# loganmcbroom/Flan

Measured on AMD Instinct MI355X. Metric: PV analysis+resynthesis frames/sec (2048-win, hop 512, 48 kHz) at 1/2/4/8 GPU, higher is better.
Workload: dtype f32; 1 GPU; 8 ch x 60 s x 48 kHz uniform noise per GPU, convert_to_PV(2048,512,dft 2048) -> convert_to_audio round trip; channels_per_gpu=8, parallelism=channel-shard x1

## Files before the change

flan_amd/__init__.py:

```python
import ctypes as C
import os

import numpy as np

_HERE = os.path.dirname(os.path.abspath(__file__))
LIB_PATH = os.environ.get("FLAN_AMD_LIB") or os.path.join(_HERE, "libflanhip.so")

OK, ERR_INVALID_ARG, ERR_UNSUPPORTED, ERR_HIP, ERR_CANCELLED, ERR_NO_DEVICE = 0, -1, -2, -3, -4, -5


class FlanHipError(RuntimeError):
    def __init__(self, code, message):
        super().__init__("flanhip error %d: %s" % (code, message))
        self.code = code


if not os.path.exists(LIB_PATH):
    raise ImportError("flan_amd/libflanhip.so is missing: build it with `python flan_amd/build.py` "
                      "(hipcc --offload-arch=gfx950); there is no fallback path")

lib = C.CDLL(LIB_PATH)

_f32p = np.ctypeslib.ndpointer(np.float32, flags="C_CONTIGUOUS")
_vp, _i64, _i32, _f32 = C.c_void_p, C.c_int64, C.c_int, C.c_float
# ... 14 lines not shown
    "flanhip_touch_pages": (C.c_int, [_vp, C.c_size_t]),
    "flanhip_host_workers": (C.c_int, []),
    "flanhip_parallel_for": (C.c_int, [C.c_int, _vp, _vp]),
    "flanhip_stream_create": (C.c_int, [C.POINTER(_vp)]),
    "flanhip_stream_destroy": (C.c_int, [_vp]),
    "flanhip_host_malloc": (C.c_int, [C.POINTER(_vp), C.c_size_t]),
    "flanhip_host_free": (C.c_int, [_vp]),
    "flanhip_memcpy_h2d": (C.c_int, [_vp, _vp, C.c_size_t, _vp]),
    "flanhip_memcpy_d2h": (C.c_int, [_vp, _vp, C.c_size_t, _vp]),
    "flanhip_memset": (C.c_int, [_vp, _i32, C.c_size_t, _vp]),
    "flanhip_stream_synchronize": (C.c_int, [_vp]),
    "flanhip_wait_cancellable": (C.c_int, [_vp, _vp]),
    "flanhip_wait_cancellable_fn": (C.c_int, [_vp, _vp, _vp]),
    "flanhip_analyze": (C.c_int, [_vp, _i64, _i64, _f32, _i32, _i32, _i32, _vp, C.POINTER(_i64), _vp]),
    "flanhip_analyze_dev": (C.c_int, [_vp, _i64, _i64, _f32, _i32, _i32, _i32, _vp, _vp]),
    "flanhip_synthesize": (C.c_int, [_vp, _i64, _i64, _i32, _f32, _f32, _i32, _vp, C.POINTER(_i32), _vp]),
    "flanhip_synthesize_workspace_bytes": (C.c_size_t, [_i64, _i64, _i32, _f32, _f32, _i32]),
    "flanhip_synthesize_dev": (C.c_int, [_vp, _i64, _i64, _i32, _f32, _f32, _i32, _vp, _vp, _vp, _vp]),
    "flanhip_analyze_dev_fused": (C.c_int, [_vp, _i64, _i64, _f32, _i32, _i32, _i32, _vp, _vp, _vp]),
    "flanhip_synthesize_dev_fused": (C.c_int, [_vp, _i64, _i64, _i32, _f32, _f32, _i32, _vp, _vp, _vp, _vp]),
    "flanhip_synthesize_dev_stages": (C.c_int, [_vp, _i64, _i64, _i32, _f32, _f32, _i32, _vp, _vp, _vp, _i32, _i32, _vp]),
    "flanhip_debug_option": (None, [_i32, _i32]),
    "flanhip_debug_kernel_scratch_bytes": (_i32, [_i32]),
    "flanhip_modify_time": (C.c_int, [_vp, _i64, _i64, _i32, _f32, _i32, _vp, _i64, _vp, _vp]),
    "flanhip_modify_time_dev": (C.c_int, [_vp, _i64, _i64, _i32, _f32, _i32, _vp, _i64, _vp, _vp]),
    "flanhip_modify_time_dev_fused": (C.c_int, [_vp, _i64, _i64, _i32, _f32, _f32, _vp, _i64, _vp, _i32, _vp, _vp]),
    "flanhip_synthesize_dev_fused_checked": (C.c_int, [_vp, _i64, _i64, _i32, _f32, _f32, _i32, _vp, _vp, _vp, _vp]),
    "flanhip_stretch_map_dev": (C.c_int, [_vp, _i64, _i32, _f32, _i32, _vp, _vp]),
    "flanhip_stretch_map_const_dev": (C.c_int, [_f32, _vp, _i64, _i32, _f32, _i32, _vp, _vp]),
    "flanhip_fill_dev": (C.c_int, [_vp, _i64, _f32, _vp]),
    "flanhip_modify_frequency": (C.c_int, [_vp, _i64, _i64, _i32, _f32, _vp, _vp, _vp, _vp]),
    "flanhip_modify_frequency_dev": (C.c_int, [_vp, _i64, _i64, _i32, _f32, _vp, _vp, _vp, _vp]),
    "flanhip_modify_time_interp_dev": (C.c_int, [_vp, _i64, _i64, _i32, _f32, _i32, _vp, _i64, _i32, _vp, _vp]),
    "flanhip_modify_time_interp_dev_fused": (C.c_int, [_vp, _i64, _i64, _i32, _f32, _f32, _vp, _i64, _i32, _vp, _i32, _vp, _vp]),
    "flanhip_modify_frequency_interp_dev": (C.c_int, [_vp, _i64, _i64, _i32, _f32, _vp, _vp, _i32, _vp, _vp]),
    "flanhip_repitch_interp_dev": (C.c_int, [_vp, _i64, _i64, _i32, _f32, _vp, _i32, _vp, _vp]),
    "flanhip_repitch_map_dev": (C.c_int, [_vp, _i64, _i64, _i32, _f32, _vp, _vp, _vp]),
    "flanhip_repitch_dev": (C.c_int, [_vp, _i64, _i64, _i32, _f32, _vp, _vp, _vp]),
    "flanhip_shape_affine": (C.c_int, [_vp, _i64, _i64, _i32, _f32, _f32, _f32, _f32, _f32, _i32, _vp, _vp]),
    "flanhip_shape_affine_dev": (C.c_int, [_vp, _i64, _i64, _i32, _f32, _f32, _f32, _f32, _f32, _i32, _vp, _vp]),
    "flanhip_shape_table_dev": (C.c_int, [_vp, _vp, _i64, _i64, _i32, _f32, _i32, _vp, _vp]),
    "flanhip_replace_amplitudes_dev": (C.c_int, [_vp, _i64, _i64, _i32, _vp, _i64, _i64, _i32, _vp, _f32, _vp, _vp]),
    "flanhip_subtract_amplitudes_dev": (C.c_int, [_vp, _i64, _i64, _i32, _vp, _i64, _i64, _i32, _vp, _f32, _vp, _vp]),
    "flanhip_resonate_out_frames": (_i64, [_i64, _f32, _f32, _i32]),
    "flanhip_resonate_dev": (C.c_int, [_vp, _i64, _i64, _i32, _f32, _i32, _i64, _vp, _f32, _vp, _vp]),
    "flanhip_n_loudest_partials_dev": (C.c_int, [_vp, _i64, _i64, _i32, _vp, C.c_int32, _i32, _vp, _vp]),
# ... 441 lines not shown


def analyze_dev(d_audio, ch, n, sample_rate, window, hop, dft, d_out, stream=None):
    check(lib.flanhip_analyze_dev(_dp(d_audio), ch, n, sample_rate, window, hop, dft, _dp(d_out), _vp(stream or 0)))


def analyze_dev_fused(d_audio, ch, n, sample_rate, window, hop, dft, d_out, d_ws, stream=None):
    check(lib.flanhip_analyze_dev_fused(_dp(d_audio), ch, n, sample_rate, window, hop, dft, _dp(d_out), _dp(d_ws), _vp(stream or 0)))


def synthesize_dev_fused(d_pv, ch, F, bins, sample_rate, analysis_rate, window, d_out, d_ws, d_nan=None, stream=None):
    check(lib.flanhip_synthesize_dev_fused(_dp(d_pv), ch, F, bins, sample_rate, analysis_rate, window, _dp(d_out), _dp(d_ws),
                                           _dp(d_nan), _vp(stream or 0)))


def synthesize_dev_stages(d_pv, ch, F, bins, sample_rate, analysis_rate, window, d_out, d_ws, d_nan, presummed, stages, stream=None):
    check(lib.flanhip_synthesize_dev_stages(_dp(d_pv), ch, F, bins, sample_rate, analysis_rate, window, _dp(d_out), _dp(d_ws),
                                            _dp(d_nan), presummed, stages, _vp(stream or 0)))


DEBUG_CHAIN_LEN, DEBUG_TARGET_CHAINS, DEBUG_FORCE_GENERIC, DEBUG_NO_FAST_DIV = 0, 1, 2, 3
DEBUG_ANA_VARIANT, DEBUG_SYN_VARIANT, DEBUG_ANA4096_OLD, DEBUG_SYN4096_OLD, DEBUG_RESAMPLE_DIRECT, DEBUG_FORCE_DIRECT, DEBUG_INLINE_FIXUP, DEBUG_WIDE_OFFSETS = 4, 5, 6, 7, 8, 9, 10, 11
_DEBUG_NAMES = {"chain_len": 0, "target_chains": 1, "force_generic": 2, "no_fast_div": 3, "ana_variant": 4, "syn_variant": 5,
                "ana4096_old": 6, "syn4096_old": 7, "resample_direct": 8, "force_direct": 9, "inline_fixup": 10, "wide_offsets": 11, "no_sub": 12}


class debug_options:

    def __init__(self, **kw):
        self.kw = {_DEBUG_NAMES[k]: int(v) for k, v in kw.items()}

    def __enter__(self):
        for k, v in self.kw.items():
            lib.flanhip_debug_option(k, v)
        return self

    def __exit__(self, *exc):
        for k in self.kw:
            lib.flanhip_debug_option(k, 0)
        return False


def synthesize_workspace_bytes(ch, F, bins, sample_rate, analysis_rate, window):
    return int(lib.flanhip_synthesize_workspace_bytes(ch, F, bins, sample_rate, analysis_rate, window))


def synthesize_dev(d_pv, ch, F, bins, sample_rate, analysis_rate, window, d_out, d_ws, d_nan=None, stream=None):
# ... 101 lines not shown
```

flan_amd/csrc/conversions.hip:

```cpp
#include "flanhip_internal.h"
#include <atomic>
#include <memory>
#include "pv_kernels.h"
#include "pv_kernels_fast.h"
#include <type_traits>
#include "pv_kernels_v2.h"
#include "pv_kernels_v3.h"
#include "pv_kernels_eo.h"
#include "pv_kernels_any.h"
#include "pv_kernels_mr.h"
#include "pv_kernels_bs.h"
#include "pv_kernels_big.h"
#include "team_launch.h"
#include "sub_launch.h"
#include <algorithm>
#include <cstdlib>

namespace flanhip {


static constexpr size_t kMaxLds = 160 * 1024;

static constexpr int kMaxAnyDft = 1 << 20;
static bool fft_size( int dft ) { return is_pow2( dft ) && dft >= 32 && dft <= 8192; }
// ... 404 lines not shown
			case 256:  return wbig ? run_synth_eo_team<4, 1, true>( p, tb, s ) : run_synth_eo_team<4, 1>( p, tb, s );
			case 512:  return wbig ? run_synth_eo_team<4, 2, true>( p, tb, s ) : run_synth_eo_team<4, 2>( p, tb, s );
			case 1024: return wbig ? run_synth_eo_team<4, 4, true>( p, tb, s ) : run_synth_eo_team<4, 4>( p, tb, s );
			}
		return FLANHIP_ERR_UNSUPPORTED;
		}
	}

static bool synth_fast_ok( int dft, int W, int hop ) { return synth_fast_kind( dft, W, hop ) != 0; }

static int self_carry_group( int dft, int W, int hop, int chains_per_channel )
	{
	if( sub_shape( dft, W, hop ) ) return chains_per_channel < 128 ? 0 : sub_group_size( dft );
	const int kind = synth_fast_kind( dft, W, hop );
	int g = 0;
	if( kind == 2 ) g = dft == 4096 ? ( debug_options().ana11_old ? 0 : 4 ) : group_size_of( dft );
	else if( kind != 1 ) return 0;
	else if( dft == 2048 || v3_size( dft ) ) g = group_size_of( dft );
	else if( dft == 4096 && !debug_options().ana11_old ) g = 4;
	if( chains_per_channel < 128 ) g = 0;
	return g;
	}

static int launch_analyze_body( const float * d_audio, int64_t ch, int64_t n, float sr, int W, int hop, int dft, flanhip_MF * d_out, void * d_fused_ws, hipStream_t s, bool * left_group_sums, int * epoch );

int launch_analyze( const float * d_audio, int64_t ch, int64_t n, float sr, int W, int hop, int dft, flanhip_MF * d_out, void * d_fused_ws, hipStream_t s )
	{
	bool left_group_sums = false;
	int epoch = 0;
	if( d_fused_ws ) note_workspace_producer( d_fused_ws, 0 );
	const int rc = launch_analyze_body( d_audio, ch, n, sr, W, hop, dft, d_out, d_fused_ws, s, &left_group_sums, &epoch );
	if( !rc && d_fused_ws && left_group_sums ) note_workspace_producer( d_fused_ws, 1, epoch );
	return rc;
	}

static int launch_analyze_body( const float * d_audio, int64_t ch, int64_t n, float sr, int W, int hop, int dft, flanhip_MF * d_out, void * d_fused_ws, hipStream_t s, bool * left_group_sums, int * epoch )
	{
	FLANHIP_REQUIRE( d_audio && d_out, FLANHIP_ERR_INVALID_ARG, "null buffer" );
	FLANHIP_REQUIRE( ch > 0 && n >= 0 && W >= 2 && hop >= 1 && sr > 0.0f, FLANHIP_ERR_INVALID_ARG, "bad sizes" );
	FLANHIP_REQUIRE( W <= dft, FLANHIP_ERR_INVALID_ARG, "window_size larger than dft_size" );
	FLANHIP_REQUIRE( dft_size_ok( dft ), FLANHIP_ERR_UNSUPPORTED, "dft_size must be even, at least 4 and at most 2^20" );
	if( int rc = require_device() ) return rc;
	const bool team = team_shape( dft, W, hop ) && n >= 2 && n < ( int64_t( 1 ) << 31 ) - 65536;
	const bool sub = sub_shape( dft, W, hop ) && n >= 2 && n < ( int64_t( 1 ) << 31 ) - 8192;
	MrPlan mr_plan{};
	const bool mr = !team && mr_size( dft, W, &mr_plan );
	BsPlan bs_plan{};
	const bool bs = !team && !mr && bs_size( dft, W, &bs_plan );
	BigPlan big_plan{};
	const bool big = !team && !mr && !bs && big_size( dft, W, &big_plan );
	const bool any = !team && !fft_size( dft ) && !mr && !bs && !big;
	std::shared_ptr<const PlanRef> plan_ref;
	if( int rc = get_plan( W, dft, &plan_ref ) ) return rc;
	const Plan * plan = &plan_ref->plan;

	AnalyzeParams p{};
	p.audio = d_audio; p.out = reinterpret_cast<MF*>( d_out );
	p.window = plan->d_window; p.tw = plan->d_tw; p.tw2 = plan->d_tw2; p.dump = plan->d_dump;
	p.n = n; p.F = n / hop + 1;
	p.num_channels = int( ch ); p.window_size = W; p.hop = hop;
	const bool fast = ( dft == 2048 || ( dft == 4096 && !debug_options().ana11_old ) || v3_size( dft ) ) && n >= 2 && n < ( int64_t( 1 ) << 31 ) - 8192 && hop <= 65536 && !force_generic();
	int target_chains = team ? team_target_chains( dft ) : sub ? sub_target_chains( dft ) : any ? any_target_chains( dft / 2 + 1 ) : mr ? mr_target_chains( dft, W ) : bs ? bs_target_chains( dft, W ) : big ? big_target_chains() : fast ? fast_target_chains( dft, false ) : generic_target_chains( dft );
	const int block_group = team ? team_group_size( dft ) : sub ? sub_group_size( dft ) : fast ? group_size_of( dft ) : 1;
	p.L = choose_chain_length( ch, p.F, any ? 7 : 1, target_chains, block_group );
	p.chains_per_channel = int( ( p.F + p.L - 1 ) / p.L );
	p.sample_rate = sr;
	p.analysis_rate = sr / hop;
	DivPlan dp;
	if( int rc = get_div_plan( p.analysis_rate, &dp ) ) return rc;
	p.ar_div = DivC{ dp.c, dp.rc, dp.exact };
	p.sums = nullptr; p.nan_out = nullptr; p.nan_epoch = 0;
	p.cancel = thread_cancel_word( s );
	bool kernel_sums = !any && !big && ( !mr || mr_pingpong( mr_plan.C ) ) && ( !bs || bs_pingpong( bs_plan.M ) );
	SynthLayout fused_lay{};
	if( d_fused_ws )
		{
		SynthLayout & lay = fused_lay;
		if( int rc = synth_layout( ch, p.F, dft / 2 + 1, sr, p.analysis_rate, W, &lay ) ) return rc;
		p.nan_epoch = next_epoch();
		*epoch = p.nan_epoch;
		if( kernel_sums && lay.L >= p.L + 8 && int64_t( p.chains_per_channel ) * ch <= target_chains ) kernel_sums = false;
		if( kernel_sums )
			{
			p.L = lay.L;
			p.chains_per_channel = lay.chains_per_channel;
			p.sums = reinterpret_cast<double*>( d_fused_ws );
			p.nan_out = reinterpret_cast<int*>( reinterpret_cast<char*>( d_fused_ws ) + lay.carry_bytes + lay.head_bytes );
			}
		const bool groups_too = ( fast || sub ) && kernel_sums && self_carry_group( dft, W, hop, lay.chains_per_channel ) != 0;
		p.group_sums = groups_too ? reinterpret_cast<double*>( reinterpret_cast<char*>( d_fused_ws ) + lay.group_offset ) : nullptr;
		p.groups_per_channel = lay.groups_per_channel;
		*left_group_sums = groups_too;
		}
	auto prepass_on_behalf = [&]() -> int
		{
		if( !d_fused_ws || kernel_sums ) return FLANHIP_OK;
		SynthParams q{};
		q.pv = reinterpret_cast<const MF*>( d_out );
		q.carry = reinterpret_cast<double*>( d_fused_ws );
		q.F = p.F; q.num_channels = int( ch ); q.num_bins = dft / 2 + 1;
		q.L = fused_lay.L; q.chains_per_channel = fused_lay.chains_per_channel;
		q.analysis_rate = p.analysis_rate; q.ar_div = p.ar_div;
		q.nan_words = reinterpret_cast<int*>( reinterpret_cast<char*>( d_fused_ws ) + fused_lay.carry_bytes + fused_lay.head_bytes );
		q.nan_epoch = p.nan_epoch;
		const int64_t chains = int64_t( q.chains_per_channel ) * ch;
		hipLaunchKernelGGL( k_phase_sums2, dim3( (unsigned) chains, (unsigned) ( ( q.num_bins + 255 ) / 256 ) ), dim3( 256 ), 0, s, q );
		FLANHIP_CHECK( hipGetLastError() );
		return FLANHIP_OK;
		};

	if( team ) { if( int rc = run_analyze_team( p, *plan, dft, s ) ) return rc; return prepass_on_behalf(); }
	if( sub ) { if( int rc = run_analyze_sub( p, dft, s ) ) return rc; return prepass_on_behalf(); }
	if( any )
		{
		std::shared_ptr<const UnitRef> unit_ref;
// ... 97 lines not shown
	FLANHIP_REQUIRE( dft_size_ok( o->dft ), FLANHIP_ERR_UNSUPPORTED, "dft size must be even, at least 4 and at most 2^20" );
	FLANHIP_REQUIRE( int64_t( o->dft ) * W < ( int64_t( 1 ) << 31 ), FLANHIP_ERR_UNSUPPORTED, "dft_size * window_size overflows the int product of AudioPV.cpp:99" );
	const bool team = team_shape( o->dft, W, o->hop );
	const bool sub = sub_shape( o->dft, W, o->hop );
	const bool mr = !team && mr_size( o->dft, W );
	const bool bs = !team && !mr && bs_size( o->dft, W );
	BigPlan big_plan{};
	o->big = !team && !mr && !bs && big_size( o->dft, W, &big_plan );
	o->any = !team && !fft_size( o->dft ) && !mr && !bs && !o->big;
	o->head_len = o->any ? 0 : std::max( W - o->hop, 0 );
	const int overlap = ( W + o->hop - 1 ) / o->hop;
	const int kind = ( o->any || o->big || sub ) ? 0 : synth_fast_kind( o->dft, W, o->hop );
	const int slots = team ? team_target_chains( o->dft ) : sub ? sub_target_chains( o->dft ) : o->any ? any_target_chains( bins ) : mr ? mr_target_chains( o->dft, W ) : bs ? bs_target_chains( o->dft, W ) : o->big ? big_target_chains() : kind == 0 ? generic_target_chains( o->dft ) : fast_target_chains( o->dft, true );
	const int block_group = team ? team_group_size( o->dft ) : sub ? sub_group_size( o->dft ) : kind != 0 ? group_size_of( o->dft ) : 1;
	o->L = choose_chain_length( ch, F, o->any ? 1 : std::max( overlap - 1, 1 ), slots, block_group );
	o->chains_per_channel = int( ( F + o->L - 1 ) / o->L );
	const int64_t chains = int64_t( o->chains_per_channel ) * ch;
	o->carry_bytes = ( size_t( chains ) * bins * sizeof( double ) + 255 ) & ~size_t( 255 );
	o->head_bytes = ( size_t( chains ) * o->head_len * sizeof( float ) + 255 ) & ~size_t( 255 );
	const int gsize = o->any ? 8 : sub ? sub_group_size( o->dft ) : group_size_of( o->dft );
	o->groups_per_channel = ( o->chains_per_channel + gsize - 1 ) / gsize;
	o->group_offset = o->carry_bytes + o->head_bytes + 1024;
	o->group_bytes = ( size_t( ch ) * o->groups_per_channel * bins * sizeof( double ) + 255 ) & ~size_t( 255 );
	o->total_bytes = o->group_offset + 2 * o->group_bytes;
	o->fix_offset = o->tail_offset = 0;
	if( ( team || ( !o->any && !mr && ( o->dft == 2048 || v3_size( o->dft ) || o->dft == 4096 ) && kind == 1 ) ) && o->head_len > 0 )
		{
		o->fix_offset = o->total_bytes;
		o->tail_offset = o->fix_offset + ( ( size_t( chains ) * 8 * sizeof( int ) + 255 ) & ~size_t( 255 ) );
		o->total_bytes = o->tail_offset + o->head_bytes;
		}
	o->any_spec_offset = o->any_frames_offset = 0;
	if( o->any )
		{
		o->any_spec_offset = o->total_bytes;
		o->any_frames_offset = o->any_spec_offset + ( ( size_t( ch ) * size_t( F ) * size_t( bins ) * sizeof( cf ) + 255 ) & ~size_t( 255 ) );
		o->total_bytes = o->any_frames_offset + ( ( size_t( ch ) * size_t( F ) * size_t( W ) * sizeof( float ) + 255 ) & ~size_t( 255 ) );
		}
	o->bsg_offset = 0;
	if( BsPlan bp{}; bs && bs_size( o->dft, W, &bp ) && bp.glob )
		{
		o->bsg_offset = o->total_bytes;
		o->total_bytes += bsg_block_bytes( bp.C, bp.M, W ) * size_t( chains );
		}
	o->mr_ring_offset = 0;
	if( MrPlan mp{}; mr && mr_size( o->dft, W, &mp ) && mp.ring_ws )
		{
// ... 55 lines not shown
	p.window_scale = 2.67f / ( lay.dft * W / lay.hop );
	DivPlan dp;
	if( int rc = get_div_plan( ar, &dp ) ) return rc;
	p.ar_div = DivC{ dp.c, dp.rc, dp.exact };
	p.dump = reinterpret_cast<float*>( reinterpret_cast<char*>( d_ws ) + lay.carry_bytes + lay.head_bytes + 512 );
	p.nan_in = ( presummed == 1 || presummed == 2 ) ? reinterpret_cast<const int*>( reinterpret_cast<char*>( d_ws ) + lay.carry_bytes + lay.head_bytes ) : nullptr;
	p.skip_words = presummed == 2 ? p.nan_in : nullptr;
	p.carry_in = d_carry_in; p.total_out = d_total_out; p.total_only = prepass_only ? 1 : 0;
	p.cancel = thread_cancel_word( s );
	const int fix_hook = debug_options().inline_fixup;
	const bool self_fix = lay.fix_offset != 0 && !prepass_only && ( stage_mask & 0xF ) == 0xF && fix_hook != 2
		&& ( fix_hook == 1 || lay.L >= ( lay.head_len + lay.hop - 1 ) / lay.hop + 3 );
	if( self_fix )
		{
		p.fix_state = reinterpret_cast<int*>( reinterpret_cast<char*>( d_ws ) + lay.fix_offset );
		p.tail = reinterpret_cast<float*>( reinterpret_cast<char*>( d_ws ) + lay.tail_offset );
		p.fix_tag = int( ( unsigned( next_epoch() ) & 0x1FFFFFFFu ) << 2 );
		}

	const int64_t chains = int64_t( p.chains_per_channel ) * ch;
	FLANHIP_REQUIRE( chains < ( int64_t( 1 ) << 31 ), FLANHIP_ERR_UNSUPPORTED, "too many chains for one launch" );
	const int stages = prepass_only ? 3 : ( stage_mask & 0xF );
	int noted_epoch = 0;
	const bool self_carry = presummed == 1 && !prepass_only && !d_carry_in && !d_total_out && debug_options().syn_variant != 2
		&& self_carry_group( lay.dft, W, lay.hop, lay.chains_per_channel ) != 0 && workspace_producer( d_ws, &noted_epoch ) == 1;
	if( self_carry )
		{
		p.expect_epoch = noted_epoch;
		p.group_sums = reinterpret_cast<const double*>( reinterpret_cast<char*>( d_ws ) + lay.group_offset );
		p.groups_per_channel = lay.groups_per_channel;
		const bool scan_groups = p.groups_per_channel > 40;
		p.group_carry = scan_groups ? reinterpret_cast<double*>( reinterpret_cast<char*>( d_ws ) + lay.group_offset + lay.group_bytes ) : nullptr;
		if( scan_groups && ( stages & 2 ) )
			{
			if( p.groups_per_channel <= 512 ) hipLaunchKernelGGL( ( k_phase_scan2<16, true> ), dim3( (unsigned) ( ( bins + 31 ) / 32 ), (unsigned) ch ), dim3( 512 ), 0, s, p );
			else hipLaunchKernelGGL( ( k_phase_scan2<32, true> ), dim3( (unsigned) ( ( bins + 15 ) / 16 ), (unsigned) ch ), dim3( 512 ), 0, s, p );
			FLANHIP_CHECK( hipGetLastError() );
			}
		}
	const int gsize = self_carry_group( lay.dft, W, lay.hop, lay.chains_per_channel );
	const bool group_kernel = !self_carry && gsize != 0 && stages == 0xF && !prepass_only && !d_carry_in && !d_total_out && debug_options().syn_variant != 2 && presummed != 3;
	const bool sums_in_group_kernel = group_kernel && presummed != 1;
	if( ( stages & 1 ) && presummed != 1 && presummed != 3 && !sums_in_group_kernel )
		{
		hipLaunchKernelGGL( k_phase_sums2, dim3( (unsigned) chains, (unsigned) ( ( bins + 255 ) / 256 ) ), dim3( 256 ), 0, s, p );
		FLANHIP_CHECK( hipGetLastError() );
		}
	if( group_kernel )
		{
		double * gs = reinterpret_cast<double*>( reinterpret_cast<char*>( d_ws ) + lay.group_offset );
		p.groups_per_channel = lay.groups_per_channel;
		const dim3 grid( (unsigned) ( ( bins + 255 ) / 256 ), (unsigned) lay.groups_per_channel, (unsigned) ch );
		FLANHIP_REQUIRE( lay.groups_per_channel <= 65535 && ch <= 65535, FLANHIP_ERR_UNSUPPORTED, "too many groups / channels for one launch" );
		if( sums_in_group_kernel ) { if( gsize == 32 ) hipLaunchKernelGGL( k_sums_and_groups<32>, grid, dim3( 256 ), 0, s, p, gs ); else if( gsize == 16 ) hipLaunchKernelGGL( k_sums_and_groups<16>, grid, dim3( 256 ), 0, s, p, gs ); else if( gsize == 8 ) hipLaunchKernelGGL( k_sums_and_groups<8>, grid, dim3( 256 ), 0, s, p, gs ); else hipLaunchKernelGGL( k_sums_and_groups<4>, grid, dim3( 256 ), 0, s, p, gs ); }
		else if( gsize == 32 ) hipLaunchKernelGGL( k_group_sums<32>, grid, dim3( 256 ), 0, s, p, gs ); else if( gsize == 16 ) hipLaunchKernelGGL( k_group_sums<16>, grid, dim3( 256 ), 0, s, p, gs ); else if( gsize == 8 ) hipLaunchKernelGGL( k_group_sums<8>, grid, dim3( 256 ), 0, s, p, gs ); else hipLaunchKernelGGL( k_group_sums<4>, grid, dim3( 256 ), 0, s, p, gs );
// ... 222 lines not shown
	{
	FLANHIP_REQUIRE( presummed >= 0 && presummed <= 2, FLANHIP_ERR_INVALID_ARG, "presummed: 0, 1 or 2" );
	return launch_synthesize( d_pv, ch, F, bins, sr, ar, W, d_out, d_ws, d_nan, presummed, (hipStream_t) stream, nullptr, nullptr, false, stages );
	}

void flanhip_debug_option( int which, int value )
	{
	DebugOptions & o = debug_options();
	switch( which )
		{
		case FLANHIP_DEBUG_CHAIN_LEN:       o.chain_len = value; break;
		case FLANHIP_DEBUG_TARGET_CHAINS:   o.target_chains = value; break;
		case FLANHIP_DEBUG_FORCE_GENERIC:   o.force_generic = value; break;
		case FLANHIP_DEBUG_NO_FAST_DIV:     o.no_fast_div = value; break;
		case FLANHIP_DEBUG_ANA_VARIANT:     o.ana_variant = value; break;
		case FLANHIP_DEBUG_SYN_VARIANT:     o.syn_variant = value; break;
		case FLANHIP_DEBUG_ANA4096_OLD:     o.ana11_old = value; break;
		case FLANHIP_DEBUG_SYN4096_OLD:     o.syn11_old = value; break;
		case FLANHIP_DEBUG_RESAMPLE_DIRECT: o.resample_direct = value; break;
		case FLANHIP_DEBUG_FORCE_DIRECT:    o.force_direct = value; break;
		case FLANHIP_DEBUG_INLINE_FIXUP:    o.inline_fixup = value; break;
		case FLANHIP_DEBUG_WIDE_OFFSETS:    o.wide_offsets = value; break;
		case FLANHIP_DEBUG_NO_SUB:          o.no_sub = value; break;
		default: break;
		}
	}
#ifdef FLANHIP_STAMPS
int flanhip_debug_read_stamps( unsigned long long * out16 )
	{
	FLANHIP_CHECK( hipDeviceSynchronize() );
	FLANHIP_CHECK( hipMemcpyFromSymbol( out16, HIP_SYMBOL( g_stamp_acc ), 16 * sizeof( unsigned long long ) ) );
	unsigned long long zero[16] = { 0 };
	FLANHIP_CHECK( hipMemcpyToSymbol( HIP_SYMBOL( g_stamp_acc ), zero, sizeof( zero ) ) );
	return FLANHIP_OK;
	}
int flanhip_debug_read_spans( unsigned long long * out8192 )
	{
	FLANHIP_CHECK( hipDeviceSynchronize() );
	FLANHIP_CHECK( hipMemcpyFromSymbol( out8192, HIP_SYMBOL( g_stamp_span ), 8192 * sizeof( unsigned long long ) ) );
	return FLANHIP_OK;
	}
#endif

size_t flanhip_synthesize_workspace_bytes( int64_t ch, int64_t F, int bins, float sr, float ar, int W )
	{
	SynthLayout lay;
	if( synth_layout( ch, F, bins, sr, ar, W, &lay ) ) return 0;
	size_t bytes = lay.total_bytes;
// ... 50 lines not shown
```

flan_amd/csrc/flanhip_internal.h:

```cpp
#pragma once
#include <hip/hip_runtime.h>
#include <cstdarg>
#include <cstdint>
#include <cstdio>
#include <cmath>
#include <map>
#include <memory>
#include <mutex>
#include <tuple>
#include <vector>

#include "flanhip.h"
#include "cf_type.h"

namespace flanhip {

void set_error( const char * fmt, ... );

#define FLANHIP_CHECK( expr )                                                                         \
	do { hipError_t e_ = ( expr );                                                                    \
		if( e_ != hipSuccess ) {                                                                      \
			::flanhip::set_error( "%s failed: %s (%s:%d)", #expr, hipGetErrorString( e_ ), __FILE__, __LINE__ ); \
			return FLANHIP_ERR_HIP; } } while( 0 )

// ... 25 lines not shown
inline int team_radix( int dft_size ) { return dft_size == 8192 ? 4 : dft_size == 16384 ? 8 : 0; }
struct TeamTableLayout { int tw1, tw3, twj, tws, two, total; };
inline TeamTableLayout team_table_layout( int R ) { TeamTableLayout l; l.tw1 = 0; l.tw3 = 240; l.twj = 1008; l.tws = l.twj + ( R - 1 ) * 512; l.two = l.tws + ( R / 2 ) * 512; l.total = l.two + 2 * R; return l; }
struct PlanRef { Plan plan; PlanRef() = default; PlanRef( const PlanRef & ) = delete; PlanRef & operator=( const PlanRef & ) = delete; ~PlanRef(); };
int get_plan( int window_size, int dft_size, std::shared_ptr<const PlanRef> * out );

struct DivPlan { float c, rc; int exact; };
int get_div_plan( float c, DivPlan * out );

int choose_chain_length( int64_t num_channels, int64_t num_frames, int min_len, int target_chains, int group = 1 );
struct DebugOptions
	{
	int chain_len = 0;
	int target_chains = 0;
	int force_generic = 0;
	int no_fast_div = 0;
	int ana_variant = 0, syn_variant = 0;
	int ana11_old = 0, syn11_old = 0;
	int resample_direct = 0;
	int wide_offsets = 0;
	int inline_fixup = 0;
	int no_sub = 0;
	int force_direct = 0;
	};
DebugOptions & debug_options();
bool force_generic();
int cu_count();

int launch_analyze( const float * d_audio, int64_t ch, int64_t n, float sr, int W, int hop, int dft, flanhip_MF * d_out, void * d_fused_ws, hipStream_t s );
int launch_synthesize( const flanhip_MF * d_pv, int64_t ch, int64_t F, int bins, float sr, float ar, int W, float * d_out,
	void * d_ws, int * d_nan, int presummed, hipStream_t s, const double * d_carry_in = nullptr, double * d_total_out = nullptr,
	bool prepass_only = false, int stage_mask = 0xF );

int next_epoch();

struct SynthLayout { int hop, dft, L, chains_per_channel, head_len, groups_per_channel; size_t carry_bytes, head_bytes, group_offset, group_bytes, total_bytes;
	size_t flags_offset;
	size_t fix_offset, tail_offset;
	bool any; size_t any_spec_offset, any_frames_offset;
	size_t mr_ring_offset;
	size_t bsg_offset;
	bool big; size_t big_out_offset, big_head_offset, big_ring_offset; };
void note_workspace_producer( const void * d_ws, int kind, int epoch = 0 );
int workspace_producer( const void * d_ws, int * epoch = nullptr );
int synth_layout( int64_t ch, int64_t F, int bins, float sr, float ar, int W, SynthLayout * out );

bool valid_interp( int kind );
float interp_eval_host( int kind, float x );
int processors_set_interp_lut( int slot, const float * d_table );
int processors_ext_set_interp_lut( int slot, const float * d_table );
int processors_arrange_set_interp_lut( int slot, const float * d_table );

}
```

flan_amd/csrc/pv_kernels.h:

```cpp
#pragma once
#include <hip/hip_runtime.h>
#include <stdint.h>
#include "fft_device.h"
#include "pv_math.h"

namespace flanhip {

struct MF { float m, f; };


struct AnalyzeParams
	{
	const float * audio;
	MF * out;
	const float * window;
	const cf * tw;
	const cf * tw2;
	int64_t n;
	int64_t F;
	int num_channels;
	int window_size;
	int hop;
	int L;
	int chains_per_channel;
	float sample_rate;
	float analysis_rate;
	DivC ar_div;
	double * sums;
	int * nan_out;
	int nan_epoch;
	double * group_sums;
	int groups_per_channel;
	const int * cancel;
	float * dump;
	};

__device__ __forceinline__ int cancel_peek( const int * word )
	{
	return word ? __hip_atomic_load( word, __ATOMIC_RELAXED, __HIP_MEMORY_SCOPE_SYSTEM ) : 0;
	}
__device__ __forceinline__ bool cancel_seen( int peeked ) { return __builtin_amdgcn_readfirstlane( peeked ) != 0; }

__device__ __forceinline__ MF phase_vocode_bin( float re, float im, float & prev_phase, float bin_frequency, float expected_phase_diff,
	float analysis_rate, bool use_wrapping )
	{
	const float phase = atan2_fast( im, re );
	const float phase_diff = phase - prev_phase;
	prev_phase = phase;
	const float delta_phase = phase_diff - expected_phase_diff;
	const float wrapped = use_wrapping ? delta_phase - FLANHIP_PI2_F * round_half_away( div_pi2( delta_phase ) ) : delta_phase;
	const float delta_frequency = div_pi2( wrapped * analysis_rate );
	MF r;
	r.m = magnitude_scaled( re, im );
	r.f = bin_frequency + delta_frequency;
	return r;
	}

// ... 440 lines not shown
```

flan_amd/csrc/pv_kernels_v2.h:

```cpp
#pragma once
#include "pv_kernels_fast.h"

namespace flanhip {

struct V2Lds
	{
	static constexpr int C = 1024;
	static constexpr int TW1 = 0;
	static constexpr int TW3 = TW1 + 240;
	static constexpr int W2H = TW3 + 768;
	static constexpr int WIN = W2H + 512;
	static constexpr int KC = WIN + 1024;
	static constexpr int BUF = KC + 1024;
	static constexpr int BUF_LEN = C + C / 16 + 1;
	static constexpr size_t bytes( int waves ) { return size_t( BUF + waves * BUF_LEN ) * 8; }
	};


#ifdef FLANHIP_STAMPS
__device__ unsigned long long g_stamp_acc[16];
__device__ unsigned long long g_stamp_span[2 * 4096];
struct Stamps
	{
	unsigned long long last, acc[12], t_begin, r_begin;
// ... 46 lines not shown
			const unsigned w = blockIdx.x * ( blockDim.x >> 6 ) + ( threadIdx.x >> 6 );
			if( w < 4096 ) { g_stamp_span[2 * w] = r_begin; g_stamp_span[2 * w + 1] = r_end; }
			}
		}
#endif
	};
#else
struct Stamps
	{
	__device__ __forceinline__ void init() {}
	__device__ __forceinline__ void operator()( int ) const {}
	__device__ __forceinline__ void flush( int ) {}
	};
#endif


#ifndef FLANHIP_PUBLISH_DRAIN
#define FLANHIP_PUBLISH_DRAIN 1
#endif
__device__ __forceinline__ void publish_drain()
	{
	if constexpr( FLANHIP_PUBLISH_DRAIN != 0 ) asm volatile( "s_waitcnt vmcnt(0)" ::: "memory" );
	else asm volatile( "" ::: "memory" );
	}

template<int WAVES, bool SUMS, int NV, int ABL = 0>
__global__ __launch_bounds__( 64 * WAVES ) void k_analyze_v2( AnalyzeParams p, FastTables tb )
	{
	using L = V2Lds;
	constexpr int C = 1024, E = 16, H = 8, NT = 64 * WAVES;
	constexpr int NP = NV / 2;
	static_assert( NV == 2 || NV == 4 || NV == 8 || NV == 16, "1, 2, 4 or 8 pairs at a time" );
	typedef float VB __attribute__(( ext_vector_type( NV ) ));
	extern __shared__ __attribute__((aligned(16))) unsigned char smem[];
	cf * s = reinterpret_cast<cf*>( smem );
	const int tid = threadIdx.x, lane = tid & 63, wave = tid >> 6;
	const int W = p.window_size, hop = p.hop;
	const int cancel_word = cancel_peek( p.cancel );

	for( int i = tid; i < 240; i += NT ) s[L::TW1 + i] = tb.tw1[i];
	for( int i = tid; i < 768; i += NT ) s[L::TW3 + i] = tb.tw3[i];
	for( int i = tid; i < 512; i += NT ) { const cf w = tb.w2[i]; s[L::W2H + i] = mk( 0.5f * w.x, 0.5f * w.y ); }
		{
		float * win = reinterpret_cast<float*>( s + L::WIN );
		for( int i = tid; i < 2 * C; i += NT ) win[i] = ( i < W ) ? p.window[i] : 0.0f;
		v4f_t * kc = reinterpret_cast<v4f_t*>( s + L::KC );
// ... 310 lines not shown
				}
			const double vx = fold( sumx );
			if( lane == 0 ) { dst[C / 2] = vx; stage[C / 2] = vx; }
			}
		const bool any_bad = __any( bad );
		if( p.nan_out && lane == 0 && active )
			{
			if( chain == 0 ) { p.nan_out[2] = p.nan_epoch; p.nan_out[4] = p.nan_epoch; }
			if( any_bad ) p.nan_out[0] = p.nan_epoch;
			}
		if( p.group_sums )
			{
			__syncthreads();
			const int live = min( WAVES, p.chains_per_channel - group * WAVES );
			double * gdst = p.group_sums + ( int64_t( channel ) * groups + group ) * ( C + 1 );
			for( int bin = tid; bin <= C; bin += NT )
				{
				double run = 0.0;
				for( int w = 0; w < live; ++w )
					{
					const double v = run + reinterpret_cast<const double*>( s + L::BUF + w * L::BUF_LEN )[bin];
					run = ( __builtin_fabs( v ) < FLANHIP_FOLD_FAST_LIMIT ) ? fold_phase_fast( v ) : fold_phase_any( v );
					}
				gdst[bin] = run;
				}
			}
		}
	}

__device__ __forceinline__ void st_agent( cf * p, cf v )
	{
	unsigned long long bits; __builtin_memcpy( &bits, &v, 8 );
	__hip_atomic_store( reinterpret_cast<unsigned long long*>( p ), bits, __ATOMIC_RELAXED, __HIP_MEMORY_SCOPE_AGENT );
	}
__device__ __forceinline__ cf ld_agent( const cf * p )
	{
	const unsigned long long bits = __hip_atomic_load( reinterpret_cast<const unsigned long long*>( p ), __ATOMIC_RELAXED, __HIP_MEMORY_SCOPE_AGENT );
	cf v; __builtin_memcpy( &v, &bits, 8 );
	return v;
	}

struct V2LdsSyn
	{
	static constexpr int C = 1024;
	static constexpr int TW1 = 0;
	static constexpr int TW3 = TW1 + 240;
	static constexpr int W2S = TW3 + 768;
// ... 464 lines not shown
```

include/flanhip.h:

```cpp
#ifndef FLANHIP_H
#define FLANHIP_H

#include <stddef.h>
#include <stdint.h>

#ifdef __cplusplus
extern "C" {
#endif

#define FLANHIP_OK                 0
#define FLANHIP_ERR_INVALID_ARG   -1
#define FLANHIP_ERR_UNSUPPORTED   -2
#define FLANHIP_ERR_HIP           -3
#define FLANHIP_ERR_CANCELLED     -4
#define FLANHIP_ERR_NO_DEVICE     -5

typedef struct flanhip_MF { float m; float f; } flanhip_MF;

int          flanhip_version(void);
const char * flanhip_last_error(void);
int          flanhip_device_count(void);
int          flanhip_set_device(int device);
int          flanhip_get_device(int * device);

// ... 42 lines not shown
                                 float sample_rate, float analysis_rate, int window_size,
                                 float * d_out, void * d_workspace, int * d_nan_flag, void * stream);
int flanhip_synthesize_dev_fused_checked(const flanhip_MF * d_pv, int64_t num_channels, int64_t num_pv_frames, int num_bins,
                                         float sample_rate, float analysis_rate, int window_size,
                                         float * d_out, void * d_workspace, int * d_nan_flag, void * stream);

int flanhip_synthesize_dev_stages(const flanhip_MF * d_pv, int64_t num_channels, int64_t num_pv_frames, int num_bins,
                                  float sample_rate, float analysis_rate, int window_size,
                                  float * d_out, void * d_workspace, int * d_nan_flag, int presummed, int stages, void * stream);

#define FLANHIP_DEBUG_CHAIN_LEN       0
#define FLANHIP_DEBUG_TARGET_CHAINS   1
#define FLANHIP_DEBUG_FORCE_GENERIC   2
#define FLANHIP_DEBUG_NO_FAST_DIV     3
#define FLANHIP_DEBUG_ANA_VARIANT     4
#define FLANHIP_DEBUG_SYN_VARIANT     5
#define FLANHIP_DEBUG_ANA4096_OLD     6
#define FLANHIP_DEBUG_SYN4096_OLD     7
#define FLANHIP_DEBUG_RESAMPLE_DIRECT 8
#define FLANHIP_DEBUG_FORCE_DIRECT    9
#define FLANHIP_DEBUG_INLINE_FIXUP   10
#define FLANHIP_DEBUG_WIDE_OFFSETS   11
#define FLANHIP_DEBUG_NO_SUB         12
void flanhip_debug_option(int which, int value);
int flanhip_debug_kernel_scratch_bytes(int which);

int flanhip_modify_time(const flanhip_MF * pv, int64_t num_channels, int64_t num_pv_frames, int num_bins,
                        float sample_rate, int hop, const float * mod_seconds,
                        int64_t out_frames, flanhip_MF * out, volatile int * cancel);
int flanhip_modify_time_dev(const flanhip_MF * d_pv, int64_t num_channels, int64_t num_pv_frames, int num_bins,
                            float sample_rate, int hop, const float * d_mod_seconds,
                            int64_t out_frames, flanhip_MF * d_out, void * stream);
int flanhip_modify_time_dev_fused(const flanhip_MF * d_pv, int64_t num_channels, int64_t num_pv_frames, int num_bins,
                                  float sample_rate, float analysis_rate, const float * d_mod, int64_t out_frames,
                                  flanhip_MF * d_out, int window_size, void * d_workspace, void * stream);
int flanhip_stretch_map_dev(float * d_factor, int64_t num_pv_frames, int num_bins, float sample_rate, int hop,
                            float * d_max, void * stream);
int flanhip_stretch_map_const_dev(float factor, float * d_map, int64_t num_pv_frames, int num_bins, float sample_rate, int hop,
                                  float * d_max, void * stream);
int flanhip_fill_dev(float * d_grid, int64_t count, float value, void * stream);

int flanhip_modify_frequency(const flanhip_MF * pv, int64_t num_channels, int64_t num_pv_frames, int num_bins,
                             float sample_rate, const float * mod_hz, const float * in_modified,
                             flanhip_MF * out, volatile int * cancel);
int flanhip_modify_frequency_dev(const flanhip_MF * d_pv, int64_t num_channels, int64_t num_pv_frames, int num_bins,
                                 float sample_rate, const float * d_mod_hz, const float * d_in_modified,
                                 flanhip_MF * d_out, void * stream);
// ... 152 lines not shown
```

Measured before the change: 168.9 million frames/s.

## Compute group phase carries in last analysis block via per-channel ticket

For dft 2048 fast path, the analysis kernel now publishes group phase sums with agent-scope stores, and a per-channel atomic ticket (epoch-tagged) picks the last-finishing block. That block scans the group sums into the carry buffer, so synthesis can skip its separate phase-scan kernel when the producer marks the workspace as carrying group carries. This trades an extra kernel launch and pass for a serial tail scan by one block per channel plus atomics and drains in analysis.

New measurement: 151.5 million frames/s. -10.3%, worse.

```diff
diff --git a/flan_amd/__init__.py b/flan_amd/__init__.py
--- a/flan_amd/__init__.py
+++ b/flan_amd/__init__.py
@@ -60,6 +60,7 @@
     "flanhip_synthesize_dev_stages": (C.c_int, [_vp, _i64, _i64, _i32, _f32, _f32, _i32, _vp, _vp, _vp, _i32, _i32, _vp]),
     "flanhip_debug_option": (None, [_i32, _i32]),
     "flanhip_debug_kernel_scratch_bytes": (_i32, [_i32]),
+    "flanhip_debug_group_layout": (C.c_int, [_i64, _i64, _i32, _f32, _f32, _i32, C.POINTER(_i64)]),
     "flanhip_modify_time": (C.c_int, [_vp, _i64, _i64, _i32, _f32, _i32, _vp, _i64, _vp, _vp]),
     "flanhip_modify_time_dev": (C.c_int, [_vp, _i64, _i64, _i32, _f32, _i32, _vp, _i64, _vp, _vp]),
     "flanhip_modify_time_dev_fused": (C.c_int, [_vp, _i64, _i64, _i32, _f32, _f32, _vp, _i64, _vp, _i32, _vp, _vp]),
@@ -547,7 +548,7 @@
 DEBUG_CHAIN_LEN, DEBUG_TARGET_CHAINS, DEBUG_FORCE_GENERIC, DEBUG_NO_FAST_DIV = 0, 1, 2, 3
 DEBUG_ANA_VARIANT, DEBUG_SYN_VARIANT, DEBUG_ANA4096_OLD, DEBUG_SYN4096_OLD, DEBUG_RESAMPLE_DIRECT, DEBUG_FORCE_DIRECT, DEBUG_INLINE_FIXUP, DEBUG_WIDE_OFFSETS = 4, 5, 6, 7, 8, 9, 10, 11
 _DEBUG_NAMES = {"chain_len": 0, "target_chains": 1, "force_generic": 2, "no_fast_div": 3, "ana_variant": 4, "syn_variant": 5,
-                "ana4096_old": 6, "syn4096_old": 7, "resample_direct": 8, "force_direct": 9, "inline_fixup": 10, "wide_offsets": 11, "no_sub": 12}
+                "ana4096_old": 6, "syn4096_old": 7, "resample_direct": 8, "force_direct": 9, "inline_fixup": 10, "wide_offsets": 11, "no_sub": 12, "group_carry": 13}
 
 
 class debug_options:
diff --git a/flan_amd/csrc/conversions.hip b/flan_amd/csrc/conversions.hip
--- a/flan_amd/csrc/conversions.hip
+++ b/flan_amd/csrc/conversions.hip
@@ -450,19 +450,19 @@
 	return g;
 	}
 
-static int launch_analyze_body( const float * d_audio, int64_t ch, int64_t n, float sr, int W, int hop, int dft, flanhip_MF * d_out, void * d_fused_ws, hipStream_t s, bool * left_group_sums, int * epoch );
+static int launch_analyze_body( const float * d_audio, int64_t ch, int64_t n, float sr, int W, int hop, int dft, flanhip_MF * d_out, void * d_fused_ws, hipStream_t s, int * left_group_sums, int * epoch );
 
 int launch_analyze( const float * d_audio, int64_t ch, int64_t n, float sr, int W, int hop, int dft, flanhip_MF * d_out, void * d_fused_ws, hipStream_t s )
 	{
-	bool left_group_sums = false;
+	int left_group_sums = 0;
 	int epoch = 0;
 	if( d_fused_ws ) note_workspace_producer( d_fused_ws, 0 );
 	const int rc = launch_analyze_body( d_audio, ch, n, sr, W, hop, dft, d_out, d_fused_ws, s, &left_group_sums, &epoch );
-	if( !rc && d_fused_ws && left_group_sums ) note_workspace_producer( d_fused_ws, 1, epoch );
+	if( !rc && d_fused_ws && left_group_sums ) note_workspace_producer( d_fused_ws, left_group_sums, epoch );
 	return rc;
 	}
 
-static int launch_analyze_body( const float * d_audio, int64_t ch, int64_t n, float sr, int W, int hop, int dft, flanhip_MF * d_out, void * d_fused_ws, hipStream_t s, bool * left_group_sums, int * epoch )
+static int launch_analyze_body( const float * d_audio, int64_t ch, int64_t n, float sr, int W, int hop, int dft, flanhip_MF * d_out, void * d_fused_ws, hipStream_t s, int * left_group_sums, int * epoch )
 	{
 	FLANHIP_REQUIRE( d_audio && d_out, FLANHIP_ERR_INVALID_ARG, "null buffer" );
 	FLANHIP_REQUIRE( ch > 0 && n >= 0 && W >= 2 && hop >= 1 && sr > 0.0f, FLANHIP_ERR_INVALID_ARG, "bad sizes" );
@@ -497,7 +497,7 @@
 	DivPlan dp;
 	if( int rc = get_div_plan( p.analysis_rate, &dp ) ) return rc;
 	p.ar_div = DivC{ dp.c, dp.rc, dp.exact };
-	p.sums = nullptr; p.nan_out = nullptr; p.nan_epoch = 0;
+	p.sums = nullptr; p.nan_out = nullptr; p.nan_epoch = 0; p.group_carry = nullptr; p.group_ticket = nullptr;
 	p.cancel = thread_cancel_word( s );
 	bool kernel_sums = !any && !big && ( !mr || mr_pingpong( mr_plan.C ) ) && ( !bs || bs_pingpong( bs_plan.M ) );
 	SynthLayout fused_lay{};
@@ -518,7 +518,10 @@
 		const bool groups_too = ( fast || sub ) && kernel_sums && self_carry_group( dft, W, hop, lay.chains_per_channel ) != 0;
 		p.group_sums = groups_too ? reinterpret_cast<double*>( reinterpret_cast<char*>( d_fused_ws ) + lay.group_offset ) : nullptr;
 		p.groups_per_channel = lay.groups_per_channel;
-		*left_group_sums = groups_too;
+		const bool carries_too = groups_too && fast && dft == 2048 && debug_options().group_carry == 0;
+		p.group_carry = carries_too ? reinterpret_cast<double*>( reinterpret_cast<char*>( d_fused_ws ) + lay.group_offset + lay.group_bytes ) : nullptr;
+		p.group_ticket = carries_too ? reinterpret_cast<unsigned long long*>( reinterpret_cast<char*>( d_fused_ws ) + lay.ticket_offset ) : nullptr;
+		*left_group_sums = groups_too ? ( carries_too ? 2 : 1 ) : 0;
 		}
 	auto prepass_on_behalf = [&]() -> int
 		{
@@ -662,7 +665,8 @@
 	o->groups_per_channel = ( o->chains_per_channel + gsize - 1 ) / gsize;
 	o->group_offset = o->carry_bytes + o->head_bytes + 1024;
 	o->group_bytes = ( size_t( ch ) * o->groups_per_channel * bins * sizeof( double ) + 255 ) & ~size_t( 255 );
-	o->total_bytes = o->group_offset + 2 * o->group_bytes;
+	o->ticket_offset = o->group_offset + 2 * o->group_bytes;
+	o->total_bytes = o->ticket_offset + ( ( size_t( ch ) * sizeof( unsigned long long ) + 255 ) & ~size_t( 255 ) );
 	o->fix_offset = o->tail_offset = 0;
 	if( ( team || ( !o->any && !mr && ( o->dft == 2048 || v3_size( o->dft ) || o->dft == 4096 ) && kind == 1 ) ) && o->head_len > 0 )
 		{
@@ -764,15 +768,18 @@
 	FLANHIP_REQUIRE( chains < ( int64_t( 1 ) << 31 ), FLANHIP_ERR_UNSUPPORTED, "too many chains for one launch" );
 	const int stages = prepass_only ? 3 : ( stage_mask & 0xF );
 	int noted_epoch = 0;
+	const int producer = workspace_producer( d_ws, &noted_epoch );
 	const bool self_carry = presummed == 1 && !prepass_only && !d_carry_in && !d_total_out && debug_options().syn_variant != 2
-		&& self_carry_group( lay.dft, W, lay.hop, lay.chains_per_channel ) != 0 && workspace_producer( d_ws, &noted_epoch ) == 1;
+		&& self_carry_group( lay.dft, W, lay.hop, lay.chains_per_channel ) != 0 && ( producer == 1 || producer == 2 );
 	if( self_carry )
 		{
 		p.expect_epoch = noted_epoch;
 		p.group_sums = reinterpret_cast<const double*>( reinterpret_cast<char*>( d_ws ) + lay.group_offset );
 		p.groups_per_channel = lay.groups_per_channel;
-		const bool scan_groups = p.groups_per_channel > 40;
-		p.group_carry = scan_groups ? reinterpret_cast<double*>( reinterpret_cast<char*>( d_ws ) + lay.group_offset + lay.group_bytes ) : nullptr;
+		const int carry_hook = debug_options().group_carry;
+		const bool carries_left = producer == 2 && lay.dft == 2048 && carry_hook == 0;
+		const bool scan_groups = !carries_left && ( p.groups_per_channel > 40 || carry_hook == 2 );
+		p.group_carry = ( carries_left || scan_groups ) ? reinterpret_cast<double*>( reinterpret_cast<char*>( d_ws ) + lay.group_offset + lay.group_bytes ) : nullptr;
 		if( scan_groups && ( stages & 2 ) )
 			{
 			if( p.groups_per_channel <= 512 ) hipLaunchKernelGGL( ( k_phase_scan2<16, true> ), dim3( (unsigned) ( ( bins + 31 ) / 32 ), (unsigned) ch ), dim3( 512 ), 0, s, p );
@@ -1041,8 +1048,18 @@
 		case FLANHIP_DEBUG_INLINE_FIXUP:    o.inline_fixup = value; break;
 		case FLANHIP_DEBUG_WIDE_OFFSETS:    o.wide_offsets = value; break;
 		case FLANHIP_DEBUG_NO_SUB:          o.no_sub = value; break;
+		case FLANHIP_DEBUG_GROUP_CARRY:     o.group_carry = value; break;
 		default: break;
 		}
+	}
+int flanhip_debug_group_layout( int64_t ch, int64_t F, int bins, float sr, float ar, int W, int64_t * out4 )
+	{
+	FLANHIP_REQUIRE( out4, FLANHIP_ERR_INVALID_ARG, "null buffer" );
+	SynthLayout lay;
+	if( int rc = synth_layout( ch, F, bins, sr, ar, W, &lay ) ) return rc;
+	out4[0] = int64_t( lay.group_offset ); out4[1] = int64_t( lay.group_offset + lay.group_bytes );
+	out4[2] = lay.groups_per_channel; out4[3] = lay.chains_per_channel;
+	return FLANHIP_OK;
 	}
 #ifdef FLANHIP_STAMPS
 int flanhip_debug_read_stamps( unsigned long long * out16 )
diff --git a/flan_amd/csrc/flanhip_internal.h b/flan_amd/csrc/flanhip_internal.h
--- a/flan_amd/csrc/flanhip_internal.h
+++ b/flan_amd/csrc/flanhip_internal.h
@@ -71,6 +71,7 @@
 	int inline_fixup = 0;
 	int no_sub = 0;
 	int force_direct = 0;
+	int group_carry = 0;
 	};
 DebugOptions & debug_options();
 bool force_generic();
@@ -84,6 +85,7 @@
 int next_epoch();
 
 struct SynthLayout { int hop, dft, L, chains_per_channel, head_len, groups_per_channel; size_t carry_bytes, head_bytes, group_offset, group_bytes, total_bytes;
+	size_t ticket_offset;
 	size_t flags_offset;
 	size_t fix_offset, tail_offset;
 	bool any; size_t any_spec_offset, any_frames_offset;
diff --git a/flan_amd/csrc/pv_kernels.h b/flan_amd/csrc/pv_kernels.h
--- a/flan_amd/csrc/pv_kernels.h
+++ b/flan_amd/csrc/pv_kernels.h
@@ -33,6 +33,8 @@
 	int groups_per_channel;
 	const int * cancel;
 	float * dump;
+	double * group_carry;
+	unsigned long long * group_ticket;
 	};
 
 __device__ __forceinline__ int cancel_peek( const int * word )
diff --git a/flan_amd/csrc/pv_kernels_v2.h b/flan_amd/csrc/pv_kernels_v2.h
--- a/flan_amd/csrc/pv_kernels_v2.h
+++ b/flan_amd/csrc/pv_kernels_v2.h
@@ -92,6 +92,18 @@
 	{
 	if constexpr( FLANHIP_PUBLISH_DRAIN != 0 ) asm volatile( "s_waitcnt vmcnt(0)" ::: "memory" );
 	else asm volatile( "" ::: "memory" );
+	}
+
+__device__ __forceinline__ void st_agent_f64( double * p, double v )
+	{
+	unsigned long long bits; __builtin_memcpy( &bits, &v, 8 );
+	__hip_atomic_store( reinterpret_cast<unsigned long long*>( p ), bits, __ATOMIC_RELAXED, __HIP_MEMORY_SCOPE_AGENT );
+	}
+__device__ __forceinline__ double ld_agent_f64( const double * p )
+	{
+	const unsigned long long bits = __hip_atomic_load( reinterpret_cast<const unsigned long long*>( p ), __ATOMIC_RELAXED, __HIP_MEMORY_SCOPE_AGENT );
+	double v; __builtin_memcpy( &v, &bits, 8 );
+	return v;
 	}
 
 template<int WAVES, bool SUMS, int NV, int ABL = 0>
@@ -448,7 +460,59 @@
 					const double v = run + reinterpret_cast<const double*>( s + L::BUF + w * L::BUF_LEN )[bin];
 					run = ( __builtin_fabs( v ) < FLANHIP_FOLD_FAST_LIMIT ) ? fold_phase_fast( v ) : fold_phase_any( v );
 					}
-				gdst[bin] = run;
+				if( p.group_carry ) st_agent_f64( gdst + bin, run ); else gdst[bin] = run;
+				}
+			if( p.group_carry )
+				{
+				asm volatile( "s_waitcnt vmcnt(0)" ::: "memory" );
+				__syncthreads();
+				int * const s_last = reinterpret_cast<int*>( smem );
+				if( tid == 0 )
+					{
+					unsigned long long * const word = p.group_ticket + channel;
+					const unsigned long long tag = static_cast<unsigned long long>( static_cast<unsigned>( p.nan_epoch ) ) << 32;
+					unsigned long long seen = __hip_atomic_load( word, __ATOMIC_RELAXED, __HIP_MEMORY_SCOPE_AGENT ), next;
+					do next = ( ( seen >> 32 ) == ( tag >> 32 ) ? seen : tag ) + 1ull;
+					while( !__hip_atomic_compare_exchange_strong( word, &seen, next, __ATOMIC_RELAXED, __ATOMIC_RELAXED, __HIP_MEMORY_SCOPE_AGENT ) );
+					*s_last = static_cast<unsigned>( next ) == static_cast<unsigned>( groups ) ? 1 : 0;
+					}
+				__syncthreads();
+				if( *s_last )
+					{
+					auto fold_syn = []( double r ) { return ( __builtin_fabs( r ) < FLANHIP_FOLD_FAST_LIMIT ) ? fold_phase_loop( r ) : fold_phase_any( r ); };
+					const double * const tot = p.group_sums + int64_t( channel ) * groups * ( C + 1 );
+					double * const car = p.group_carry + int64_t( channel ) * groups * ( C + 1 );
+					auto scan_bins = [&]( int bin0, int bin1, bool has0, bool has1 )
+						{
+						constexpr int KEEP = 32;
+						double run0 = 0.0, run1 = 0.0;
+						for( int g0 = 0; g0 < groups; g0 += KEEP )
+							{
+							double v0[KEEP], v1[KEEP];
+							#pragma unroll
+							for( int u = 0; u < KEEP; ++u )
+								{
+								v0[u] = ( g0 + u < groups ) ? ld_agent_f64( tot + int64_t( g0 + u ) * ( C + 1 ) + bin0 ) : 0.0;
+								v1[u] = ( g0 + u < groups ) ? ld_agent_f64( tot + int64_t( g0 + u ) * ( C + 1 ) + bin1 ) : 0.0;
+								}
+							#pragma unroll
+							for( int u = 0; u < KEEP; ++u )
+								{
+								if( g0 + u < groups )
+									{
+									const bool padded = ( ( g0 + u ) & 15 ) != 0;
+									if( has0 ) car[int64_t( g0 + u ) * ( C + 1 ) + bin0] = padded ? fold_syn( run0 + 0.0 ) : run0;
+									if( has1 ) car[int64_t( g0 + u ) * ( C + 1 ) + bin1] = padded ? fold_syn( run1 + 0.0 ) : run1;
+									run0 = fold_syn( run0 + v0[u] );
+									run1 = fold_syn( run1 + v1[u] );
+									}
+								}
+							}
+						};
+					static_assert( NT == C / 2, "two bins per thread, bin C on its own" );
+					scan_bins( tid, tid + NT, true, true );
+					if( wave == 1 ) scan_bins( C, C, lane == 0, false );
+					}
 				}
 			}
 		}
diff --git a/include/flanhip.h b/include/flanhip.h
--- a/include/flanhip.h
+++ b/include/flanhip.h
@@ -88,7 +88,9 @@
 #define FLANHIP_DEBUG_INLINE_FIXUP   10
 #define FLANHIP_DEBUG_WIDE_OFFSETS   11
 #define FLANHIP_DEBUG_NO_SUB         12
+#define FLANHIP_DEBUG_GROUP_CARRY    13
 void flanhip_debug_option(int which, int value);
+int flanhip_debug_group_layout(int64_t num_channels, int64_t num_pv_frames, int num_bins, float sample_rate, float analysis_rate, int window_size, int64_t * out4);
 int flanhip_debug_kernel_scratch_bytes(int which);
 
 int flanhip_modify_time(const flanhip_MF * pv, int64_t num_channels, int64_t num_pv_frames, int num_bins,
```
